# ETH3D/dataset-pipeline

Hardware: AMD Instinct MI355X
Metric: ICP correspondences/sec (higher is better)
Workload: dtype f32 (f64 accumulation); 1 GPU; ICPScanAligner 2 scans x 50000000 points, -d 0.01 (BASELINE.json configs[1] shape), one outer iteration per step; scans=2, parallelism=dp1

## Files before the change

### dataset-pipeline_amd/csrc/e3d_icp.hip

```cpp
#include <atomic>
#include <algorithm>
#include <cfloat>
#include <chrono>
#include <cmath>
#include <condition_variable>
#include <cstdio>
#include <functional>
#include <map>
#include <memory>
#include <mutex>
#include <thread>

#include "../../include/e3d_hip.h"
#include "e3d_comm.hpp"
#include "e3d_icp_kernels.hpp"
#include "e3d_math.hpp"

#pragma clang fp contract(off)

namespace e3d {

static thread_local std::string g_last_error;
void set_last_error(const std::string& msg) { g_last_error = msg; }
const char* last_error_cstr() { return g_last_error.c_str(); }
// ... 123 lines not shown
  bool stop_ = false;
};

}

using namespace e3d;

struct e3d_icp {
  int device = 0;
  hipStream_t stream = nullptr;
  std::vector<std::unique_ptr<Cloud>> clouds;
  std::unique_ptr<Cloud> fixed;
  int max_inner = 150;
  bool sequential_dsum = env_default_off("E3D_ICP_SEQUENTIAL_DISTANCE_SUM");
  DevBuf<float> d2_by_orig;
  std::vector<float> h_d2_by_orig;
  int nn_mode = 0;
  size_t dense_cell_budget = [] { const char* e = getenv("E3D_DENSE_CELLS"); return e ? (size_t)strtoull(e, nullptr, 10) : (size_t)1 << 33; }();
  int rank = 0, world = 1;
  e3d_allreduce_fn allreduce = nullptr;
  void* allreduce_user = nullptr;
  e3d_comm* comm = nullptr;
  DevBuf<double> d_red;

  DevBuf<float> bbox_partial, bbox_out;
  PinBuf<float> h_bbox;
  DevBuf<unsigned long long> keys_a, keys_b;
  DevBuf<unsigned> vals_a, vals_b, counter;
  DevBuf<char> sort_temp;
  DevBuf<int> match_pos;
  DevBuf<float> match_d2;
  DevBuf<unsigned> block_counts, block_offsets, block_groups, chunk_groups;
  DevBuf<unsigned char> block_done;
  DevBuf<double> block_d2, chunk_d2;
  DevBuf<unsigned long long> d_total, chunk_sum;
  DevBuf<double> d_total_d2;
  PinBuf<unsigned long long> h_total;
  PinBuf<double> h_total_d2;
  DevBuf<float4> cA, cB, cC;
  size_t corr_used = 0;
  bool resident_rows = env_default_on("E3D_ICP_RESIDENT");
  bool resident_now = false;
  int lm_prev_end_step = -1;
  std::unique_ptr<SolvePool> solve_pool;
  DevBuf<LmSet> d_sets;
  PinBuf<LmSet> h_sets;
  DevBuf<LmPose> d_poses;
  PinBuf<LmPose> h_poses;
  DevBuf<int> d_block_set;
  DevBuf<double> d_partial, d_setsum;
  PinBuf<double> h_setsum;
  std::unique_ptr<EventTimer> lm_timer, nn_timer, nn_timer_c;
  struct LazyTimer {
    std::vector<std::pair<hipEvent_t, hipEvent_t>> ev;
    size_t used = 0;
    double acc = 0.0;
    void start(hipStream_t s) {
      if (used == ev.size()) { hipEvent_t a, b; E3D_HIP(hipEventCreate(&a)); E3D_HIP(hipEventCreate(&b)); ev.emplace_back(a, b); }
      E3D_HIP(hipEventRecord(ev[used].first, s));
    }
    void stop(hipStream_t s) { E3D_HIP(hipEventRecord(ev[used].second, s)); ++used; }
    double take() {
      for (size_t i = 0; i < used; ++i) {
        float t = 0.f;
        if (hipEventSynchronize(ev[i].second) == hipSuccess && hipEventElapsedTime(&t, ev[i].first, ev[i].second) == hipSuccess) acc += (double)t;
      }
// ... 459 lines not shown
  if (kept == 0) return 0;
  if (k32) sort_pairs_u32_u32(reinterpret_cast<unsigned*>(h->keys_a.p), reinterpret_cast<unsigned*>(h->keys_b.p), h->vals_a.p, h->vals_b.p, kept, tgt.key_bits, h->sort_temp, s, n);
  else sort_pairs_u64_u32(h->keys_a.p, h->keys_b.p, h->vals_a.p, h->vals_b.p, kept, tgt.key_bits, h->sort_temp, s, n);
  return kept;
}

static double g_nn_prof[8];
static bool nn_profile() { static const bool on = env_default_off("E3D_NN_PROFILE"); return on; }
struct NnPhase {
  hipStream_t s; int slot; std::chrono::steady_clock::time_point t0;
  NnPhase(hipStream_t st, int sl) : s(st), slot(sl) { if (nn_profile()) { (void)hipStreamSynchronize(s); t0 = std::chrono::steady_clock::now(); } }
  ~NnPhase() { if (nn_profile()) { (void)hipStreamSynchronize(s); g_nn_prof[slot] += std::chrono::duration<double, std::milli>(std::chrono::steady_clock::now() - t0).count(); } }
};

static bool pair_is_dense(const e3d_icp* h, const Cloud& tgt) {
  return h->nn_mode >= 2 || (h->nn_mode == 0 && (double)tgt.n >= 4.0 * (double)std::max(tgt.n_cells, 1u));
}
static bool pair_uses_rows(const e3d_icp* h, const Cloud& tgt) {
  return pair_is_dense(h, tgt) && tgt.has_dense && (h->nn_mode == 0 || h->nn_mode == 3 || h->nn_mode == 5);
}
static bool far_list_is_short(size_t n_far, size_t n) {
  static const long long div = [] { const char* e = getenv("E3D_NN_FAR_DIV"); return e ? atoll(e) : 32ll; }();
  return n_far > 0 && (div <= 0 || n_far * (size_t)div < n);
}
static size_t resident_rows_cap(size_t n) { return div_up(n, 64) * 64; }
static size_t resident_bytes(size_t n) { return resident_rows_cap(n) * 48 + n * 4 + div_up(n, 64) * 4; }

struct BatchItem {
  PairJob* job; Cloud* src; Cloud* tgt; size_t j0, n; PairState* ps;
  InvMap im; CertParams cert; BoundParams bp; double cum_pair;
  MotionBound cum_up;
  float near2; bool none_near;
  bool certified = false, from_state = false; size_t n_near = 0, n_far = 0;
};

static void prepare_pair(BatchItem& it, float d) {
  const NnSwitches& sw = nn_switches();
  const Cloud& src = *it.src; const Cloud& tgt = *it.tgt;
  const PairState& ps = *it.ps;
  it.im = make_invmap(tgt);
  it.cum_pair = src.cum_motion + tgt.cum_motion;
  MotionBound m_lo;
  pair_motion_bounds(ps, src, tgt, m_lo, it.cum_up);
  it.cert = make_cert_params(tgt, m_lo);
  it.n_far = it.n; it.n_near = 0;
  it.certified = !ps.fresh && sw.use_cert && certify_now(ps, src, tgt);
  it.from_state = !ps.fresh && sw.use_cert && !it.certified;
  it.near2 = (float)((sw.near_frac * (double)d) * (sw.near_frac * (double)d));
  it.none_near = sw.np_frac > 0 && (src.last_motion + tgt.last_motion) < sw.np_gate * (double)d;
  double smin = cloud_smin(tgt);
  if (!(smin > 1e-12)) smin = 1e-12;
  double m_local = 0;
  for (int k = 0; k < 3; ++k) m_local = std::max(m_local, std::max(std::fabs((double)tgt.lmin[k]), std::fabs((double)tgt.lmax[k])));
  it.bp.margin = (float)(sw.margin_frac * (double)d);
  it.bp.rho_scale = round_up_f((1.0 + 1e-5) / smin);
  it.bp.rho_pad = round_up_f(2.0 * tgt.build_slack + 8.0 * FLT_EPSILON * m_local);
  it.bp.lo = it.cert.lo;
  it.bp.cell_scale = it.cert.cell_scale; it.bp.cell_sub = it.cert.cell_sub;
  it.bp.np_extra = it.none_near ? (float)(sw.np_frac * (double)d) : 0.f;
}

static void search_bounded_lists(e3d_icp* h, BatchItem& it, const unsigned* todo_near, const unsigned* todo_far, float* match_d2, float d, e3d_icp_iter_record& rec) {
  hipStream_t s = h->stream;
  const Cloud& tgt = *it.tgt;
  PairState& ps = *it.ps;
  const float4* srcG = it.src->G4.p + it.j0;
// ... 270 lines not shown
    launch_corr_totals(n, h->block_counts.p, h->block_d2.p, h->block_groups.p, h->chunk_sum.p, h->chunk_d2.p, h->chunk_groups.p,
                       h->d_totals_all.p + 3 * i, h->d_d2_all.p + i, ps.glist.p, s);
    h->tm_scan.stop(s);
    rec.nn_update_launches++; rec.nn_kernel_launches += 4;
  }
  read_back_batch(h, items, rec);
}

static bool find_pairs_multi(e3d_icp* h, std::vector<BatchItem>& items, float d, e3d_icp_iter_record& rec) {
  hipStream_t s = h->stream;
  const size_t B = items.size();
  for (const BatchItem& it : items) if (!it.tgt->has_half || h->nn_mode == 5) return false;
  const NnSwitches& sw = nn_switches();
  while (h->slots.size() < B) h->slots.emplace_back(new e3d_icp::PairSlot());
  h->h_todo_all.reserve(2 * kPairBatch); h->d_todo_all.reserve(2 * kPairBatch);
  h->d_totals_all.reserve(3 * kPairBatch); h->d_d2_all.reserve(kPairBatch); h->h_totals_all.reserve(3 * kPairBatch); h->h_d2_all.reserve(kPairBatch);
  h->h_batch.reserve(1); h->d_batch.reserve(1);
  NnBatchDev& T = h->h_batch.p[0];
  static_assert(kPairBatch <= (size_t)kNnBatchPairs, "pair table too small");
  T.n_pairs = (int)B; T.n_jobs = 0;
  unsigned cert_blocks = 0, upd_blocks = 0, chunks = 0;
  long long cert_queries = 0;
  E3D_HIP(hipMemsetAsync(h->d_todo_all.p, 0, 2 * sizeof(unsigned) * B, s));
  for (size_t i = 0; i < B; ++i) {
    BatchItem& it = items[i];
    e3d_icp::PairSlot& sl = *h->slots[i];
    Cloud& src = *it.src; Cloud& tgt = *it.tgt;
    PairState& ps = *it.ps;
    const size_t n = it.n;
    sl.match_d2.reserve(n); sl.todo_near.reserve(n); sl.todo_far.reserve(n);
    prepare_pair(it, d);
    const RowFrames rf = ensure_resident_rows(ps, src, tgt, n, s);
    const bool sg = rf.sg, tg = rf.tg;
    NnPairDev& P = T.pair[i];
    P.Gsrc = src.G4.p + it.j0; P.Gtgt = tgt.G4.p; P.S = tgt.dense_start.p; P.H8 = tgt.half_prefix.p;
    P.match = ps.match.p; P.match2 = ps.match2.p; P.lbe = ps.lbe.p; P.match_d2 = sl.match_d2.p;
    P.todo_near = sl.todo_near.p; P.todo_far = sl.todo_far.p; P.counts = h->d_todo_all.p + 2 * i;
    P.n = (unsigned)n; P.none_near = it.none_near ? 1 : 0;
    P.cum_up = it.cum_up;
    P.near2 = it.near2;
    P.g = tgt.grid; P.im = it.im; P.qr = tgt.qrange; P.bp = it.bp;
    P.Psrc = (sg ? src.G4.p : src.L4.p) + it.j0; P.LNsrc = src.LN.p + it.j0; P.Ptgt = tg ? tgt.G4.p : tgt.L4.p; P.LNtgt = tgt.LN.p;
    P.src_global = sg ? 1 : 0; P.tgt_global = tg ? 1 : 0; P.Tsrc = to_affine(src.T); P.Ttgt = to_affine(tgt.T);
    P.A = ps.pA.p; P.B = ps.pB.p; P.C = ps.pC.p; P.plane_match = ps.plane_match.p; P.glist = ps.glist.p;
    if (it.certified) { cert_blocks += (unsigned)div_up(n, (size_t)kNnCertBlockQueries); cert_queries += (long long)n; }
    T.cert_end[i] = cert_blocks;
    const unsigned nb = (unsigned)div_up(n, kBlock);
    upd_blocks += nb; T.upd_end[i] = upd_blocks;
    chunks += (unsigned)div_up((size_t)nb, (size_t)kNnScanChunk); T.chunk_end[i] = chunks;
  }
  h->block_counts.reserve(upd_blocks); h->block_d2.reserve(upd_blocks); h->block_groups.reserve(upd_blocks);
  h->chunk_sum.reserve(chunks + 1); h->chunk_d2.reserve(chunks + 1); h->chunk_groups.reserve(chunks + 1); h->chunk_rewritten.reserve(chunks + 1);
  {
    if (sw.fuse_update && cert_blocks) { h->block_done.reserve(upd_blocks); E3D_HIP(hipMemsetAsync(h->block_done.p, 0, upd_blocks, s)); }
    unsigned b0 = 0;
    for (size_t i = 0; i < B; ++i) {
      NnPairDev& P = T.pair[i];
      const bool on = sw.fuse_update && cert_blocks && items[i].certified && (1.0 - items[i].ps->settled_frac) < sw.fuse_gate;
      P.upd_counts = on ? h->block_counts.p + b0 : nullptr; P.upd_d2 = on ? h->block_d2.p + b0 : nullptr;
      P.upd_groups = on ? h->block_groups.p + b0 : nullptr; P.upd_done = on ? h->block_done.p + b0 : nullptr;
      b0 = T.upd_end[i];
    }
  }
  E3D_HIP(hipMemcpyAsync(h->d_batch.p, h->h_batch.p, sizeof(NnBatchDev), hipMemcpyHostToDevice, s));
  if (cert_blocks) {
    h->tm_certify.start(s);
    launch_nn_certify_multi(h->d_batch.p, cert_blocks, radius_sq(d), s);
    h->tm_certify.stop(s);
    rec.nn_certify_launches++; rec.nn_certify_queries += cert_queries; rec.nn_kernel_launches++;
    copy_out(h->h_todo_all.p, h->d_todo_all.p, 2 * sizeof(unsigned) * B, s);
  }
  sync(h);
  unsigned job_blocks = 0;
  long long job_queries = 0;
  for (size_t i = 0; i < B; ++i) {
    BatchItem& it = items[i];
    if (!it.certified) continue;
    e3d_icp::PairSlot& sl = *h->slots[i];
    it.n_near = h->h_todo_all.p[2 * i]; it.n_far = h->h_todo_all.p[2 * i + 1];
    certify_ran(*it.ps, *it.src, *it.tgt, it.n, it.n_near + it.n_far);
    auto add_job = [&](const unsigned* list, size_t n_list) {
      if (!n_list) return;
      const int jb = T.n_jobs++;
      T.job_pair[jb] = (int)i; T.job_list[jb] = list; T.job_n[jb] = (unsigned)n_list;
      job_blocks += (unsigned)div_up(n_list, kBlock); T.job_end[jb] = job_blocks;
      job_queries += (long long)n_list;
    };
    add_job(sl.todo_near.p, it.n_near);
    if (far_list_is_short(it.n_far, it.n)) {
      add_job(sl.todo_far.p, it.n_far);
      it.n_near += it.n_far; it.n_far = 0;
    }
  }
  auto launch_bounded_jobs = [&] {
    if (T.n_jobs <= 0) return;
    E3D_HIP(hipMemcpyAsync(h->d_batch.p, h->h_batch.p, sizeof(NnBatchDev), hipMemcpyHostToDevice, s));
    h->tm_bounded.start(s);
    launch_nn_bounded_half_multi(h->d_batch.p, job_blocks, radius_sq(d), s);
    h->tm_bounded.stop(s);
    rec.nn_bounded_launches++; rec.nn_bounded_queries += job_queries; rec.nn_kernel_launches++;
  };
  auto seeds_for = [&](const BatchItem& it) { return sw.seed_allowed && it.n_far > 0 && (it.ps->fresh ? sw.seed_fresh : it.ps->matched_frac >= sw.seed_frac); };
  size_t far_pairs = 0, far_total = 0;
  int kb_max = 1;
  for (size_t i = 0; i < B; ++i) if (items[i].n_far > 0) { ++far_pairs; far_total += items[i].n_far; kb_max = std::max(kb_max, items[i].tgt->key_bits); }
// ... 960 lines not shown
```

### dataset-pipeline_amd/csrc/e3d_icp_kernels.hip

```cpp
#include <cstdlib>

#include "e3d_icp_kernels.hpp"

#pragma clang fp contract(off)

namespace e3d {

__global__ __launch_bounds__(kBlock) void k_transform_aos(const float* __restrict__ xyz,
                                                          const float* __restrict__ nrm, size_t n, Affine T,
                                                          float* __restrict__ oxyz, float* __restrict__ onrm,
                                                          float* __restrict__ bbox_partial) {
  float mn[3] = {3.402823466e+38f, 3.402823466e+38f, 3.402823466e+38f};
  float mx[3] = {-3.402823466e+38f, -3.402823466e+38f, -3.402823466e+38f};
  for (size_t i = (size_t)blockIdx.x * blockDim.x + threadIdx.x; i < n; i += (size_t)gridDim.x * blockDim.x) {
    const float x = xyz[3 * i], y = xyz[3 * i + 1], z = xyz[3 * i + 2];
    const float3 p = pcl_se3(T, x, y, z);
    oxyz[3 * i] = p.x; oxyz[3 * i + 1] = p.y; oxyz[3 * i + 2] = p.z;
    if (nrm) {
      const float3 q = pcl_so3(T, nrm[3 * i], nrm[3 * i + 1], nrm[3 * i + 2]);
      onrm[3 * i] = q.x; onrm[3 * i + 1] = q.y; onrm[3 * i + 2] = q.z;
    }
    mn[0] = fminf(mn[0], p.x); mn[1] = fminf(mn[1], p.y); mn[2] = fminf(mn[2], p.z);
    mx[0] = fmaxf(mx[0], p.x); mx[1] = fmaxf(mx[1], p.y); mx[2] = fmaxf(mx[2], p.z);
  }
// ... 1074 lines not shown
        for (int r = 0; r < 9; ++r) {
          if (Q[G].bt - p < rl[r]) lb_pos = (int)(rs[r] + (Q[G].bt - p));
          p += rl[r];
        }
      }
      float lb_d2 = Q[G].bd; unsigned lb_oi = Q[G].boi;
      {
        const float od2 = __shfl_xor(lb_d2, 32, 64);
        const unsigned ooi = (unsigned)__shfl_xor((int)lb_oi, 32, 64);
        const int opos = __shfl_xor(lb_pos, 32, 64);
        if (od2 < lb_d2 || (od2 == lb_d2 && ooi < lb_oi)) { lb_d2 = od2; lb_oi = ooi; lb_pos = opos; }
      }
      const float sd2 = __shfl(lb_d2, slot_of_lane & 31, 64);
      const unsigned soi = (unsigned)__shfl((int)lb_oi, slot_of_lane & 31, 64);
      const int spos = __shfl(lb_pos, slot_of_lane & 31, 64);
      if ((slot_of_lane >> 5) == G) { rd2 = sd2; roi = soi; rpos = spos; }
    }
    if ((seg >> lane) & 1ull) {
      if (rd2 < best_d2 || (rd2 == best_d2 && roi < best_oi)) { best_d2 = rd2; best_oi = roi; best_pos = rpos; }
    }
    remaining &= ~seg;
  }
  if (valid) { match_pos[pos] = best_pos; match_d2[pos] = best_d2; }
}

constexpr int kCertPerWave = 512;
template <int kCertUnroll>
__device__ __forceinline__ void nn_certify_body(const unsigned bx, const float4* __restrict__ Gsrc, size_t n, const float4* __restrict__ Gtgt,
                                                const MotionBound cum_up, float r2, float near2, int none_near, int* __restrict__ match,
                                                int* __restrict__ match2, const float* __restrict__ lbe,
                                                float* __restrict__ match_d2, unsigned* __restrict__ todo_near,
                                                unsigned* __restrict__ todo_far, unsigned* __restrict__ counts,
                                                unsigned* __restrict__ upd_counts = nullptr, double* __restrict__ upd_d2 = nullptr,
                                                unsigned* __restrict__ upd_groups = nullptr, unsigned char* __restrict__ upd_done = nullptr) {
  __shared__ unsigned s_list[2][kBlock / kWave][kCertPerWave];
  __shared__ unsigned s_cnt[2][kBlock / kWave];
  __shared__ unsigned s_base[2];
  const int lane = threadIdx.x & 63, w = threadIdx.x >> 6;
  const size_t j0 = ((size_t)bx * (kBlock / kWave) + (size_t)w) * kCertPerWave;
  unsigned cn = 0, cf = 0;
  for (int step0 = 0; step0 < kCertPerWave / kWave; step0 += kCertUnroll) {
    size_t jj[kCertUnroll];
    bool vv[kCertUnroll];
    int mm[kCertUnroll], mm2[kCertUnroll];
    float ll[kCertUnroll];
    float4 qq[kCertUnroll], c1[kCertUnroll], c2v[kCertUnroll];
#pragma unroll
    for (int u = 0; u < kCertUnroll; ++u) {
      jj[u] = j0 + (size_t)(step0 + u) * kWave + (size_t)lane;
      vv[u] = jj[u] < n;
      const size_t js = vv[u] ? jj[u] : 0;
      mm[u] = ld_stream(match + js); mm2[u] = ld_stream(match2 + js); ll[u] = ld_stream(lbe + js); qq[u] = ld_stream(Gsrc + js);
    }
#pragma unroll
    for (int u = 0; u < kCertUnroll; ++u) {
      c1[u] = Gtgt[mm[u] >= 0 ? mm[u] : 0];
      c2v[u] = Gtgt[(mm[u] >= 0 && mm2[u] >= 0) ? mm2[u] : 0];
    }
    unsigned ub_c = 0, ub_g = 0, ub_gm = 0;
    double ub_t = 0.0;
    bool ub_bad = false;
    static_assert(kCertUnroll == 4, "four steps of 64 queries = one block of the row update");
#pragma unroll
    for (int u = 0; u < kCertUnroll; ++u) {
    const size_t j = jj[u];
    const bool valid = vv[u];
    bool ok = false, near = false;
    bool swapped = false;
    float v_ok = 0.f;
    if (valid) {
      const float thr = (ll[u] - motion_up(qq[u], cum_up)) * 0.999999f;
      const float lim = thr * thr * 0.999999f;
      const int m = mm[u];
      if (m >= 0) {
        const int m2 = mm2[u];
        const float4 q = qq[u];
        const float4 c = c1[u];
        float v = sqdist_l2(q.x, q.y, q.z, c.x, c.y, c.z);
        if (m2 >= 0) {
          const float4 c2 = c2v[u];
          const float v2 = sqdist_l2(q.x, q.y, q.z, c2.x, c2.y, c2.z);
          if (v2 < v || (v2 == v && __float_as_uint(c2.w) < __float_as_uint(c.w))) {
            v = v2;
            if (thr > 0.f && v < lim && v < r2) { match[j] = m2; match2[j] = m; swapped = true; }
          }
        }
        ok = (thr > 0.f) && (v < lim) && (v < r2);
        near = v < near2;
        if (ok) { st_stream(match_d2 + j, v); v_ok = v; }
      } else {
        ok = (thr > 0.f) && (lim >= r2);
        near = none_near != 0;
        st_stream(match_d2 + j, r2);
      }
    }
    const unsigned long long fn = __ballot(valid && !ok && near), ff = __ballot(valid && !ok && !near);
    const unsigned long long below = (1ull << lane) - 1ull;
    if (valid && !ok) {
      if (near) s_list[0][w][cn + (unsigned)__popcll(fn & below)] = (unsigned)j;
      else s_list[1][w][cf + (unsigned)__popcll(ff & below)] = (unsigned)j | (mm[u] < 0 ? kListNoPartner : 0u);
    }
    cn += (unsigned)__popcll(fn); cf += (unsigned)__popcll(ff);
    if (upd_done) {
      const bool f = valid && mm[u] >= 0;
      const unsigned gc = (unsigned)__popcll(__ballot(f));
      const double gd = wave_sum((f && ok) ? (double)v_ok : 0.0);
      ub_c += gc; ub_t += gd;
      if (gc) { ++ub_g; ub_gm |= 1u << u; }
      if (__ballot(valid && (!ok || swapped))) ub_bad = true;
    }
    }
    if (upd_done) {
      const size_t blk = j0 / kBlock + (size_t)(step0 / kCertUnroll);
      if (blk < (n + kBlock - 1) / kBlock && lane == 0) {
        if (!ub_bad) { upd_counts[blk] = ub_c; upd_d2[blk] = ub_t; upd_groups[blk] = ub_g | (ub_gm << 8); }
        upd_done[blk] = ub_bad ? 0 : 1;
      }
    }
  }
  if (lane == 0) { s_cnt[0][w] = cn; s_cnt[1][w] = cf; }
  __syncthreads();
  if (threadIdx.x < 2) {
    unsigned tot = 0;
    for (int k = 0; k < kBlock / kWave; ++k) tot += s_cnt[threadIdx.x][k];
    s_base[threadIdx.x] = tot ? atomicAdd(&counts[threadIdx.x], tot) : 0u;
  }
  __syncthreads();
  unsigned bn = s_base[0], bf = s_base[1];
  for (int k = 0; k < w; ++k) { bn += s_cnt[0][k]; bf += s_cnt[1][k]; }
  for (unsigned i = (unsigned)lane; i < cn; i += kWave) todo_near[bn + i] = s_list[0][w][i];
  for (unsigned i = (unsigned)lane; i < cf; i += kWave) todo_far[bf + i] = s_list[1][w][i];
}

template <int kCertUnroll>
__global__ __launch_bounds__(kBlock) void k_nn_certify(const float4* __restrict__ Gsrc, size_t n, const float4* __restrict__ Gtgt,
                                                       MotionBound cum_up, float r2, float near2, int none_near, int* __restrict__ match,
                                                       int* __restrict__ match2, const float* __restrict__ lbe,
                                                       float* __restrict__ match_d2, unsigned* __restrict__ todo_near,
                                                       unsigned* __restrict__ todo_far, unsigned* __restrict__ counts) {
  nn_certify_body<kCertUnroll>(blockIdx.x, Gsrc, n, Gtgt, cum_up, r2, near2, none_near, match, match2, lbe, match_d2, todo_near, todo_far, counts);
}

__device__ __forceinline__ int nn_find_range(const unsigned* __restrict__ ends, int n, unsigned b) {
  int lo = 0, hi = n - 1;
  while (lo < hi) {
    const int mid = (lo + hi) >> 1;
    if (b < ends[mid]) hi = mid; else lo = mid + 1;
  }
  return __builtin_amdgcn_readfirstlane(lo);
}

__global__ __launch_bounds__(kBlock) void k_nn_certify_multi(const NnBatchDev* __restrict__ B, float r2) {
  const int p = nn_find_range(B->cert_end, B->n_pairs, blockIdx.x);
  const unsigned bx = blockIdx.x - (p ? B->cert_end[p - 1] : 0u);
  const NnPairDev& P = B->pair[p];
  nn_certify_body<4>(bx, P.Gsrc, (size_t)P.n, P.Gtgt, P.cum_up, r2, P.near2, P.none_near, P.match, P.match2, P.lbe, P.match_d2,
                     P.todo_near, P.todo_far, P.counts, P.upd_counts, P.upd_d2, P.upd_groups, P.upd_done);
}

template <int LPQ>
__global__ __launch_bounds__(kBlock) void k_nn_bounded(const float4* __restrict__ Gsrc, const unsigned* __restrict__ list,
                                                       unsigned n_list, const float4* __restrict__ Gtgt, const unsigned* __restrict__ S,
                                                       GridDesc g, InvMap im, QueryRange qr, float r2, BoundParams bp,
                                                       int* __restrict__ match, int* __restrict__ match2,
                                                       float* __restrict__ match_d2, float* __restrict__ lbe) {
  const unsigned i = (blockIdx.x * blockDim.x + threadIdx.x) / LPQ;
  const int sub = threadIdx.x % LPQ;
  if (i >= n_list) return;
  const unsigned j = list[i] & kListIndexMask;
  const float4 q = Gsrc[j];
  const int m = match[j];
  float d1 = r2;
  if (m >= 0) {
    const float4 pc = Gtgt[m];
    d1 = sqdist_l2(q.x, q.y, q.z, pc.x, pc.y, pc.z);
    const int m2 = match2[j];
    if (m2 >= 0) { const float4 pc2 = Gtgt[m2]; d1 = fminf(d1, sqdist_l2(q.x, q.y, q.z, pc2.x, pc2.y, pc2.z)); }
  }
  const float dr = sqrtf(fminf(d1, r2)) + ((m < 0) ? bp.np_extra : bp.margin);
  const float cover2 = (d1 < r2) ? fminf(dr * dr * 1.000001f, r2) : ((m < 0) ? dr * dr * 1.000001f : r2);
  const float rho = sqrtf(cover2) * bp.rho_scale + bp.rho_pad;
  const float dx = q.x - im.t[0], dy = q.y - im.t[1], dz = q.z - im.t[2];
  const float lx = im.Linv[0] * dx + im.Linv[1] * dy + im.Linv[2] * dz;
  const float ly = im.Linv[3] * dx + im.Linv[4] * dy + im.Linv[5] * dz;
  const float lz = im.Linv[6] * dx + im.Linv[7] * dy + im.Linv[8] * dz;
  const int x0 = max(cell_coord(lx - rho, g.origin[0], g.inv_cell) - qr.lo[0], 0), x1 = min(cell_coord(lx + rho, g.origin[0], g.inv_cell) - qr.lo[0], (int)qr.D[0] - 1);
  const int y0 = max(cell_coord(ly - rho, g.origin[1], g.inv_cell) - qr.lo[1], 0), y1 = min(cell_coord(ly + rho, g.origin[1], g.inv_cell) - qr.lo[1], (int)qr.D[1] - 1);
  const int z0 = max(cell_coord(lz - rho, g.origin[2], g.inv_cell) - qr.lo[2], 0), z1 = min(cell_coord(lz + rho, g.origin[2], g.inv_cell) - qr.lo[2], (int)qr.D[2] - 1);
  const float kInf = __uint_as_float(0x7f800000u);
  float cover_box2 = 0.f;
// ... 620 lines not shown
                                                         float4* __restrict__ C, size_t out_base) {
  const size_t j = (size_t)blockIdx.x * blockDim.x + threadIdx.x;
  const int m = (j < n) ? ld_stream(match_pos + j) : -1;
  const bool f = m >= 0;
  const unsigned long long b = __ballot(f);
  __shared__ unsigned wbase[kBlock / kWave];
  const int lane = threadIdx.x & 63, w = threadIdx.x >> 6;
  if (lane == 0) wbase[w] = (unsigned)__popcll(b);
  __syncthreads();
  unsigned base = block_offsets[blockIdx.x];
  for (int k = 0; k < w; ++k) base += wbase[k];
  if (!f) return;
  const unsigned rank = (unsigned)__popcll(b & ((1ull << lane) - 1ull));
  const size_t o = out_base + base + rank;
  const size_t js = order ? (size_t)ld_stream(order + j) : j;
  const float4 sp = order ? Gsrc[js] : ld_stream(Gsrc + js);
  const float4 ln = order ? LNsrc[js] : ld_stream(LNsrc + js);
  const float3 sn = pcl_so3(Tsrc, ln.x, ln.y, ln.z);
  const float4 tp = Gtgt[m];
  const float4 tl = LNtgt[m];
  const float3 tn = pcl_so3(Ttgt, tl.x, tl.y, tl.z);
  st_stream(A + o, make_float4(sp.x, sp.y, sp.z, sn.x));
  st_stream(B + o, make_float4(sn.y, sn.z, tp.x, tp.y));
  st_stream(C + o, make_float4(tp.z, tn.x, tn.y, tn.z));
}

__device__ __forceinline__ void corr_update_body(const unsigned bx, const int* __restrict__ match, int* __restrict__ plane_match,
                                                 const float* __restrict__ match_d2, size_t n,
                                                 const float4* __restrict__ Psrc, const float4* __restrict__ LNsrc,
                                                 const int src_global, const Affine& Tsrc, const float4* __restrict__ Ptgt,
                                                 const float4* __restrict__ LNtgt, const int tgt_global, const Affine& Ttgt,
                                                 float4* __restrict__ A, float4* __restrict__ B, float4* __restrict__ C,
                                                 unsigned* __restrict__ block_counts, double* __restrict__ block_d2,
                                                 unsigned* __restrict__ block_groups, const unsigned char* __restrict__ done = nullptr) {
  if (done && done[bx]) return;
  const size_t j = (size_t)bx * blockDim.x + threadIdx.x;
  const bool in = j < n;
  const int m = in ? ld_stream(match + j) : -1;
  const int pm = in ? ld_stream(plane_match + j) : -1;
  const bool f = m >= 0;
  const unsigned long long chg = __ballot(in && m != pm);
  const bool wr = in && (((chg >> (threadIdx.x & 56)) & 0xFFull) != 0ull);
  const unsigned long long wrb = __ballot(wr);
  if (wr) {
    float4 ra = make_float4(0.f, 0.f, 0.f, 0.f), rb = ra, rc = ra;
    if (f) {
      const float4 sp = Psrc[j];
      const float4 ln = LNsrc[j];
      float3 sn = make_float3(ln.x, ln.y, ln.z);
      if (src_global) sn = pcl_so3(Tsrc, ln.x, ln.y, ln.z);
      const float4 tp = Ptgt[m];
      const float4 tl = LNtgt[m];
      float3 tn = make_float3(tl.x, tl.y, tl.z);
      if (tgt_global) tn = pcl_so3(Ttgt, tl.x, tl.y, tl.z);
      ra = make_float4(sp.x, sp.y, sp.z, sn.x);
      rb = make_float4(sn.y, sn.z, tp.x, tp.y);
      rc = make_float4(tp.z, tn.x, tn.y, tn.z);
    }
    st_stream(A + j, ra); st_stream(B + j, rb); st_stream(C + j, rc);
    if (m != pm) plane_match[j] = m;
  }
  const unsigned long long b = __ballot(f);
  double d = f ? (double)ld_stream(match_d2 + j) : 0.0;
  d = wave_sum(d);
  __shared__ unsigned sc[kBlock / kWave], sw[kBlock / kWave];
  __shared__ double sd[kBlock / kWave];
  if ((threadIdx.x & 63) == 0) { sc[threadIdx.x >> 6] = (unsigned)__popcll(b); sw[threadIdx.x >> 6] = (unsigned)__popcll(wrb); sd[threadIdx.x >> 6] = d; }
  __syncthreads();
  if (threadIdx.x == 0) {
    unsigned c = 0, g = 0, gm = 0, rw = 0; double t = 0;
    for (int k = 0; k < kBlock / kWave; ++k) { c += sc[k]; t += sd[k]; rw += sw[k]; if (sc[k]) { ++g; gm |= 1u << k; } }
    block_counts[bx] = c; block_d2[bx] = t; block_groups[bx] = g | (gm << 8) | (rw << 16);
  }
}

__global__ __launch_bounds__(kBlock) void k_corr_update(const int* __restrict__ match, int* __restrict__ plane_match,
                                                        const float* __restrict__ match_d2, size_t n,
                                                        const float4* __restrict__ Psrc, const float4* __restrict__ LNsrc,
                                                        const int src_global, Affine Tsrc, const float4* __restrict__ Ptgt,
                                                        const float4* __restrict__ LNtgt, const int tgt_global, Affine Ttgt,
                                                        float4* __restrict__ A, float4* __restrict__ B, float4* __restrict__ C,
                                                        unsigned* __restrict__ block_counts, double* __restrict__ block_d2,
                                                        unsigned* __restrict__ block_groups) {
  corr_update_body(blockIdx.x, match, plane_match, match_d2, n, Psrc, LNsrc, src_global, Tsrc, Ptgt, LNtgt, tgt_global, Ttgt, A, B, C,
                   block_counts, block_d2, block_groups);
}

__global__ __launch_bounds__(kBlock) void k_corr_update_multi(const NnBatchDev* __restrict__ Bt, unsigned* __restrict__ block_counts,
                                                              double* __restrict__ block_d2, unsigned* __restrict__ block_groups) {
  const int p = nn_find_range(Bt->upd_end, Bt->n_pairs, blockIdx.x);
  const unsigned b0 = p ? Bt->upd_end[p - 1] : 0u;
  const NnPairDev& P = Bt->pair[p];
  const Affine Ts = P.Tsrc, Tt = P.Ttgt;
  corr_update_body(blockIdx.x - b0, P.match, P.plane_match, P.match_d2, (size_t)P.n, P.Psrc, P.LNsrc, P.src_global, Ts, P.Ptgt, P.LNtgt,
                   P.tgt_global, Tt, P.A, P.B, P.C, block_counts + b0, block_d2 + b0, block_groups + b0, P.upd_done);
}

__device__ __forceinline__ void group_list_body(const unsigned bx, const unsigned* __restrict__ block_groups, int nblocks,
                                                const unsigned* __restrict__ chunk_gbase, unsigned* __restrict__ glist) {
  const int b = (int)bx * kScanChunk + threadIdx.x;
  const unsigned w = (b < nblocks) ? block_groups[b] : 0u;
  const unsigned c = w & 0xFFu;
  const int lane = threadIdx.x & 63, wv = threadIdx.x >> 6;
  unsigned inc = c;
#pragma unroll
  for (int o = 1; o < 64; o <<= 1) {
    const unsigned t = __shfl_up(inc, o, 64);
    if (lane >= o) inc += t;
  }
  __shared__ unsigned ws[kScanChunk / kWave];
  if (lane == 63) ws[wv] = inc;
  __syncthreads();
  unsigned base = chunk_gbase[bx] + (inc - c);
  for (int k = 0; k < wv; ++k) base += ws[k];
  const unsigned mask = w >> 8;
#pragma unroll
  for (int k = 0; k < kBlock / kWave; ++k)
    if (mask & (1u << k)) glist[base++] = (unsigned)b * (kBlock / kWave) + (unsigned)k;
}

__global__ __launch_bounds__(kScanChunk) void k_group_list(const unsigned* __restrict__ block_groups, int nblocks,
                                                           const unsigned* __restrict__ chunk_gbase,
                                                           unsigned* __restrict__ glist) {
  group_list_body(blockIdx.x, block_groups, nblocks, chunk_gbase, glist);
}

__global__ __launch_bounds__(kScanChunk) void k_scan_chunk_sums_multi(const NnBatchDev* __restrict__ Bt, const unsigned* __restrict__ block_counts,
                                                                      const double* __restrict__ block_d2, const unsigned* __restrict__ block_groups,
// ... 874 lines not shown
```

### dataset-pipeline_amd/csrc/e3d_icp_kernels.hpp

```cpp
#pragma once

#include <functional>

#include "e3d_common.hpp"
#include "e3d_kernels.hpp"

namespace e3d {

enum { kModeCost = 0,
       kModeOne = 1,
       kModeTwo = 2,
       kModeTwoCross = 3
};
constexpr int kLmMaxPoses = 10;
constexpr int kLmSlot = 91;
constexpr int kMaxBboxBlocks = 2048;
constexpr int kRowCap = 128;
constexpr unsigned kListNoPartner = 0x80000000u, kListIndexMask = 0x7FFFFFFFu;
constexpr int kRowSpan = 4;
constexpr int kNNCap = 256;

struct QueryRange { int lo[3]; unsigned D[3]; };

struct LmSet {
// ... 61 lines not shown
  float rho_scale;
  float rho_pad;
  MotionBound lo;
  float cell_scale, cell_sub;
  float np_extra;
};
void launch_nn_bounded(const float4* Gsrc, const unsigned* list, size_t n_list, const float4* Gtgt, const unsigned* dense_start,
                       const unsigned long long* half_prefix, bool half_always, const GridDesc& g, const InvMap& im, const QueryRange& qr, float r2,
                       const BoundParams& bp, int* match, int* match2, float* match_d2, float* lbe, hipStream_t s);
constexpr int kNnBatchPairs = 32;
constexpr int kNnBatchJobs = 2 * kNnBatchPairs;
struct NnPairDev {
  const float4* Gsrc;
  const float4* Gtgt;
  const unsigned* S;
  const unsigned long long* H8;
  int *match, *match2;
  float* lbe;
  float* match_d2;
  unsigned *todo_near, *todo_far;
  unsigned* counts;
  unsigned n;
  int none_near;
  MotionBound cum_up;
  float near2;
  GridDesc g; InvMap im; QueryRange qr; BoundParams bp;
  const float4 *Psrc, *LNsrc, *Ptgt, *LNtgt;
  int src_global, tgt_global;
  Affine Tsrc, Ttgt;
  float4 *A, *B, *C;
  int* plane_match;
  unsigned* glist;
  unsigned* upd_counts; double* upd_d2; unsigned* upd_groups; unsigned char* upd_done;
  const unsigned* far_list;
  const unsigned* occ;
  unsigned far_n, occ_stride;
  int far_flags;
  unsigned rows_off, rows_n;
  unsigned* seed_list;
  float seed2;
};
constexpr unsigned kQueryKeysBlock = 2048;
constexpr unsigned kQuerySeedBlock = 1024;
struct NnBatchDev {
  int n_pairs, n_jobs;
  int key_shift;
  unsigned far_end[kNnBatchPairs];
  unsigned rows_end[kNnBatchPairs];
  unsigned cert_end[kNnBatchPairs];
  unsigned upd_end[kNnBatchPairs];
  unsigned chunk_end[kNnBatchPairs];
  unsigned job_end[kNnBatchJobs];
  int job_pair[kNnBatchJobs];
  unsigned job_n[kNnBatchJobs];
  const unsigned* job_list[kNnBatchJobs];
  NnPairDev pair[kNnBatchPairs];
};
void launch_nn_certify_multi(const NnBatchDev* batch, unsigned n_blocks, float r2, hipStream_t s);
void launch_nn_bounded_half_multi(const NnBatchDev* batch, unsigned n_blocks, float r2, hipStream_t s);
void launch_query_keys_multi(bool keys32, const NnBatchDev* batch, unsigned n_blocks, float r2, void* keys, unsigned* vals, unsigned* counts, hipStream_t s);
void launch_query_seed_multi(bool keys32, const NnBatchDev* batch, unsigned n_blocks, float r2, void* keys, unsigned* vals, unsigned* counts, hipStream_t s);
void launch_nn_rows_multi(const NnBatchDev* batch, unsigned n_blocks, const unsigned* order, float r2, hipStream_t s);
void launch_corr_update_multi(const NnBatchDev* batch, unsigned n_blocks, unsigned* block_counts, double* block_d2, unsigned* block_groups, hipStream_t s);
void launch_corr_totals_multi(const NnBatchDev* batch, int n_pairs, unsigned n_chunks, const unsigned* block_counts, const double* block_d2,
                              const unsigned* block_groups, unsigned long long* chunk_sum, double* chunk_d2, unsigned* chunk_groups,
                              unsigned* chunk_rewritten, unsigned long long* totals, double* total_d2, hipStream_t s);
// ... 43 lines not shown
```

Measured before the change: 6.719 billion correspondences/s.

## Settle fused row-update work per wave instead of per block

The certify kernel now records which of the four 64-query waves in a row-update block are settled, storing per-wave counts and d2 sums for partially settled blocks instead of marking the whole block unsettled. The row-update kernel skips loads and stores for settled waves and reads their precomputed stats, so mixed blocks do less work. It also disables fusion for pairs whose resident rows were just reset, and adds an optional stats dump of how many blocks are settled whole or mixed. This costs extra scratch buffers and per-wave branching inside the update kernel.

```diff
diff --git a/dataset-pipeline_amd/csrc/e3d_icp.hip b/dataset-pipeline_amd/csrc/e3d_icp.hip
--- a/dataset-pipeline_amd/csrc/e3d_icp.hip
+++ b/dataset-pipeline_amd/csrc/e3d_icp.hip
@@ -179,6 +179,8 @@
   DevBuf<float> match_d2;
   DevBuf<unsigned> block_counts, block_offsets, block_groups, chunk_groups;
   DevBuf<unsigned char> block_done;
+  DevBuf<unsigned> block_gcnt;
+  DevBuf<double> block_gd2;
   DevBuf<double> block_d2, chunk_d2;
   DevBuf<unsigned long long> d_total, chunk_sum;
   DevBuf<double> d_total_d2;
@@ -704,6 +706,7 @@
   MotionBound cum_up;
   float near2; bool none_near;
   bool certified = false, from_state = false; size_t n_near = 0, n_far = 0;
+  bool rows_reset = false;
 };
 
 static void prepare_pair(BatchItem& it, float d) {
@@ -1040,6 +1043,7 @@
     prepare_pair(it, d);
     const RowFrames rf = ensure_resident_rows(ps, src, tgt, n, s);
     const bool sg = rf.sg, tg = rf.tg;
+    it.rows_reset = rf.reset;
     NnPairDev& P = T.pair[i];
     P.Gsrc = src.G4.p + it.j0; P.Gtgt = tgt.G4.p; P.S = tgt.dense_start.p; P.H8 = tgt.half_prefix.p;
     P.match = ps.match.p; P.match2 = ps.match2.p; P.lbe = ps.lbe.p; P.match_d2 = sl.match_d2.p;
@@ -1060,13 +1064,17 @@
   h->block_counts.reserve(upd_blocks); h->block_d2.reserve(upd_blocks); h->block_groups.reserve(upd_blocks);
   h->chunk_sum.reserve(chunks + 1); h->chunk_d2.reserve(chunks + 1); h->chunk_groups.reserve(chunks + 1); h->chunk_rewritten.reserve(chunks + 1);
   {
-    if (sw.fuse_update && cert_blocks) { h->block_done.reserve(upd_blocks); E3D_HIP(hipMemsetAsync(h->block_done.p, 0, upd_blocks, s)); }
+    if (sw.fuse_update && cert_blocks) {
+      h->block_done.reserve(upd_blocks); h->block_gcnt.reserve(upd_blocks); h->block_gd2.reserve(4 * (size_t)upd_blocks);
+      E3D_HIP(hipMemsetAsync(h->block_done.p, 0, upd_blocks, s));
+    }
     unsigned b0 = 0;
     for (size_t i = 0; i < B; ++i) {
       NnPairDev& P = T.pair[i];
-      const bool on = sw.fuse_update && cert_blocks && items[i].certified && (1.0 - items[i].ps->settled_frac) < sw.fuse_gate;
+      const bool on = sw.fuse_update && cert_blocks && items[i].certified && !items[i].rows_reset && (1.0 - items[i].ps->settled_frac) < sw.fuse_gate;
       P.upd_counts = on ? h->block_counts.p + b0 : nullptr; P.upd_d2 = on ? h->block_d2.p + b0 : nullptr;
       P.upd_groups = on ? h->block_groups.p + b0 : nullptr; P.upd_done = on ? h->block_done.p + b0 : nullptr;
+      P.upd_gcnt = on ? h->block_gcnt.p + b0 : nullptr; P.upd_gd2 = on ? h->block_gd2.p + 4 * (size_t)b0 : nullptr;
       b0 = T.upd_end[i];
     }
   }
@@ -1079,6 +1087,23 @@
     copy_out(h->h_todo_all.p, h->d_todo_all.p, 2 * sizeof(unsigned) * B, s);
   }
   sync(h);
+  if (sw.want_stats && sw.fuse_update && cert_blocks) {
+    std::vector<unsigned char> masks(upd_blocks);
+    E3D_HIP(hipMemcpyAsync(masks.data(), h->block_done.p, upd_blocks, hipMemcpyDeviceToHost, s));
+    sync(h);
+    unsigned b0 = 0;
+    for (size_t i = 0; i < B; ++i) {
+      unsigned whole = 0, mixed = 0, groups = 0;
+      for (unsigned b = b0; b < T.upd_end[i]; ++b) {
+        const unsigned m = masks[b];
+        if (m == 0xFu) ++whole; else if (m) ++mixed;
+        groups += (unsigned)__builtin_popcount(m);
+      }
+      if (T.pair[i].upd_done)
+        fprintf(stderr, "[fuse %d->%d] blocks %u settled whole %u mixed %u settled groups %u\n", items[i].job->src, items[i].job->tgt, T.upd_end[i] - b0, whole, mixed, groups);
+      b0 = T.upd_end[i];
+    }
+  }
   unsigned job_blocks = 0;
   long long job_queries = 0;
   for (size_t i = 0; i < B; ++i) {
diff --git a/dataset-pipeline_amd/csrc/e3d_icp_kernels.hip b/dataset-pipeline_amd/csrc/e3d_icp_kernels.hip
--- a/dataset-pipeline_amd/csrc/e3d_icp_kernels.hip
+++ b/dataset-pipeline_amd/csrc/e3d_icp_kernels.hip
@@ -1130,7 +1130,8 @@
                                                 float* __restrict__ match_d2, unsigned* __restrict__ todo_near,
                                                 unsigned* __restrict__ todo_far, unsigned* __restrict__ counts,
                                                 unsigned* __restrict__ upd_counts = nullptr, double* __restrict__ upd_d2 = nullptr,
-                                                unsigned* __restrict__ upd_groups = nullptr, unsigned char* __restrict__ upd_done = nullptr) {
+                                                unsigned* __restrict__ upd_groups = nullptr, unsigned char* __restrict__ upd_done = nullptr,
+                                                unsigned* __restrict__ upd_gcnt = nullptr, double* __restrict__ upd_gd2 = nullptr) {
   __shared__ unsigned s_list[2][kBlock / kWave][kCertPerWave];
   __shared__ unsigned s_cnt[2][kBlock / kWave];
   __shared__ unsigned s_base[2];
@@ -1155,9 +1156,8 @@
       c1[u] = Gtgt[mm[u] >= 0 ? mm[u] : 0];
       c2v[u] = Gtgt[(mm[u] >= 0 && mm2[u] >= 0) ? mm2[u] : 0];
     }
-    unsigned ub_c = 0, ub_g = 0, ub_gm = 0;
-    double ub_t = 0.0;
-    bool ub_bad = false;
+    unsigned ub_m = 0, ub_pc = 0;
+    double ub_d[kCertUnroll];
     static_assert(kCertUnroll == 4, "four steps of 64 queries = one block of the row update");
 #pragma unroll
     for (int u = 0; u < kCertUnroll; ++u) {
@@ -1199,20 +1199,33 @@
       else s_list[1][w][cf + (unsigned)__popcll(ff & below)] = (unsigned)j | (mm[u] < 0 ? kListNoPartner : 0u);
     }
     cn += (unsigned)__popcll(fn); cf += (unsigned)__popcll(ff);
-    if (upd_done) {
+    ub_d[u] = 0.0;
+    if (upd_done && !__ballot(valid && (!ok || swapped))) {
       const bool f = valid && mm[u] >= 0;
-      const unsigned gc = (unsigned)__popcll(__ballot(f));
-      const double gd = wave_sum((f && ok) ? (double)v_ok : 0.0);
-      ub_c += gc; ub_t += gd;
-      if (gc) { ++ub_g; ub_gm |= 1u << u; }
-      if (__ballot(valid && (!ok || swapped))) ub_bad = true;
+      ub_pc |= (unsigned)__popcll(__ballot(f)) << (8 * u);
+      ub_d[u] = wave_sum(f ? (double)v_ok : 0.0);
+      ub_m |= 1u << u;
     }
     }
     if (upd_done) {
       const size_t blk = j0 / kBlock + (size_t)(step0 / kCertUnroll);
       if (blk < (n + kBlock - 1) / kBlock && lane == 0) {
-        if (!ub_bad) { upd_counts[blk] = ub_c; upd_d2[blk] = ub_t; upd_groups[blk] = ub_g | (ub_gm << 8); }
-        upd_done[blk] = ub_bad ? 0 : 1;
+        if (ub_m == 0xFu) {
+          unsigned c = 0, g = 0, gm = 0; double t = 0;
+#pragma unroll
+          for (int u = 0; u < kCertUnroll; ++u) {
+            const unsigned gc = (ub_pc >> (8 * u)) & 0xFFu;
+            c += gc; t += ub_d[u];
+            if (gc) { ++g; gm |= 1u << u; }
+          }
+          upd_counts[blk] = c; upd_d2[blk] = t; upd_groups[blk] = g | (gm << 8);
+        } else if (ub_m) {
+          upd_gcnt[blk] = ub_pc;
+#pragma unroll
+          for (int u = 0; u < kCertUnroll; ++u)
+            if (ub_m & (1u << u)) upd_gd2[4 * blk + (size_t)u] = ub_d[u];
+        }
+        upd_done[blk] = (unsigned char)ub_m;
       }
     }
   }
@@ -1253,7 +1266,7 @@
   const unsigned bx = blockIdx.x - (p ? B->cert_end[p - 1] : 0u);
   const NnPairDev& P = B->pair[p];
   nn_certify_body<4>(bx, P.Gsrc, (size_t)P.n, P.Gtgt, P.cum_up, r2, P.near2, P.none_near, P.match, P.match2, P.lbe, P.match_d2,
-                     P.todo_near, P.todo_far, P.counts, P.upd_counts, P.upd_d2, P.upd_groups, P.upd_done);
+                     P.todo_near, P.todo_far, P.counts, P.upd_counts, P.upd_d2, P.upd_groups, P.upd_done, P.upd_gcnt, P.upd_gd2);
 }
 
 template <int LPQ>
@@ -1940,40 +1953,47 @@
                                                  const float4* __restrict__ LNtgt, const int tgt_global, const Affine& Ttgt,
                                                  float4* __restrict__ A, float4* __restrict__ B, float4* __restrict__ C,
                                                  unsigned* __restrict__ block_counts, double* __restrict__ block_d2,
-                                                 unsigned* __restrict__ block_groups, const unsigned char* __restrict__ done = nullptr) {
-  if (done && done[bx]) return;
-  const size_t j = (size_t)bx * blockDim.x + threadIdx.x;
-  const bool in = j < n;
-  const int m = in ? ld_stream(match + j) : -1;
-  const int pm = in ? ld_stream(plane_match + j) : -1;
-  const bool f = m >= 0;
-  const unsigned long long chg = __ballot(in && m != pm);
-  const bool wr = in && (((chg >> (threadIdx.x & 56)) & 0xFFull) != 0ull);
-  const unsigned long long wrb = __ballot(wr);
-  if (wr) {
-    float4 ra = make_float4(0.f, 0.f, 0.f, 0.f), rb = ra, rc = ra;
-    if (f) {
-      const float4 sp = Psrc[j];
-      const float4 ln = LNsrc[j];
-      float3 sn = make_float3(ln.x, ln.y, ln.z);
-      if (src_global) sn = pcl_so3(Tsrc, ln.x, ln.y, ln.z);
-      const float4 tp = Ptgt[m];
-      const float4 tl = LNtgt[m];
-      float3 tn = make_float3(tl.x, tl.y, tl.z);
-      if (tgt_global) tn = pcl_so3(Ttgt, tl.x, tl.y, tl.z);
-      ra = make_float4(sp.x, sp.y, sp.z, sn.x);
-      rb = make_float4(sn.y, sn.z, tp.x, tp.y);
-      rc = make_float4(tp.z, tn.x, tn.y, tn.z);
-    }
-    st_stream(A + j, ra); st_stream(B + j, rb); st_stream(C + j, rc);
-    if (m != pm) plane_match[j] = m;
-  }
-  const unsigned long long b = __ballot(f);
-  double d = f ? (double)ld_stream(match_d2 + j) : 0.0;
-  d = wave_sum(d);
+                                                 unsigned* __restrict__ block_groups, const unsigned char* __restrict__ done = nullptr,
+                                                 const unsigned* __restrict__ gcnt = nullptr, const double* __restrict__ gd2 = nullptr) {
+  const unsigned settled = done ? (unsigned)done[bx] : 0u;
+  if (settled == 0xFu) return;
   __shared__ unsigned sc[kBlock / kWave], sw[kBlock / kWave];
   __shared__ double sd[kBlock / kWave];
-  if ((threadIdx.x & 63) == 0) { sc[threadIdx.x >> 6] = (unsigned)__popcll(b); sw[threadIdx.x >> 6] = (unsigned)__popcll(wrb); sd[threadIdx.x >> 6] = d; }
+  const int wv = __builtin_amdgcn_readfirstlane((int)(threadIdx.x >> 6));
+  if ((settled >> wv) & 1u) {
+    if ((threadIdx.x & 63) == 0) { sc[wv] = (gcnt[bx] >> (8 * wv)) & 0xFFu; sw[wv] = 0u; sd[wv] = gd2[4 * (size_t)bx + (size_t)wv]; }
+  } else {
+    const size_t j = (size_t)bx * blockDim.x + threadIdx.x;
+    const bool in = j < n;
+    const int m = in ? ld_stream(match + j) : -1;
+    const int pm = in ? ld_stream(plane_match + j) : -1;
+    const bool f = m >= 0;
+    const unsigned long long chg = __ballot(in && m != pm);
+    const bool wr = in && (((chg >> (threadIdx.x & 56)) & 0xFFull) != 0ull);
+    const unsigned long long wrb = __ballot(wr);
+    if (wr) {
+      float4 ra = make_float4(0.f, 0.f, 0.f, 0.f), rb = ra, rc = ra;
+      if (f) {
+        const float4 sp = Psrc[j];
+        const float4 ln = LNsrc[j];
+        float3 sn = make_float3(ln.x, ln.y, ln.z);
+        if (src_global) sn = pcl_so3(Tsrc, ln.x, ln.y, ln.z);
+        const float4 tp = Ptgt[m];
+        const float4 tl = LNtgt[m];
+        float3 tn = make_float3(tl.x, tl.y, tl.z);
+        if (tgt_global) tn = pcl_so3(Ttgt, tl.x, tl.y, tl.z);
+        ra = make_float4(sp.x, sp.y, sp.z, sn.x);
+        rb = make_float4(sn.y, sn.z, tp.x, tp.y);
+        rc = make_float4(tp.z, tn.x, tn.y, tn.z);
+      }
+      st_stream(A + j, ra); st_stream(B + j, rb); st_stream(C + j, rc);
+      if (m != pm) plane_match[j] = m;
+    }
+    const unsigned long long b = __ballot(f);
+    double d = f ? (double)ld_stream(match_d2 + j) : 0.0;
+    d = wave_sum(d);
+    if ((threadIdx.x & 63) == 0) { sc[wv] = (unsigned)__popcll(b); sw[wv] = (unsigned)__popcll(wrb); sd[wv] = d; }
+  }
   __syncthreads();
   if (threadIdx.x == 0) {
     unsigned c = 0, g = 0, gm = 0, rw = 0; double t = 0;
@@ -2001,7 +2021,7 @@
   const NnPairDev& P = Bt->pair[p];
   const Affine Ts = P.Tsrc, Tt = P.Ttgt;
   corr_update_body(blockIdx.x - b0, P.match, P.plane_match, P.match_d2, (size_t)P.n, P.Psrc, P.LNsrc, P.src_global, Ts, P.Ptgt, P.LNtgt,
-                   P.tgt_global, Tt, P.A, P.B, P.C, block_counts + b0, block_d2 + b0, block_groups + b0, P.upd_done);
+                   P.tgt_global, Tt, P.A, P.B, P.C, block_counts + b0, block_d2 + b0, block_groups + b0, P.upd_done, P.upd_gcnt, P.upd_gd2);
 }
 
 __device__ __forceinline__ void group_list_body(const unsigned bx, const unsigned* __restrict__ block_groups, int nblocks,
diff --git a/dataset-pipeline_amd/csrc/e3d_icp_kernels.hpp b/dataset-pipeline_amd/csrc/e3d_icp_kernels.hpp
--- a/dataset-pipeline_amd/csrc/e3d_icp_kernels.hpp
+++ b/dataset-pipeline_amd/csrc/e3d_icp_kernels.hpp
@@ -117,6 +117,7 @@
   int* plane_match;
   unsigned* glist;
   unsigned* upd_counts; double* upd_d2; unsigned* upd_groups; unsigned char* upd_done;
+  unsigned* upd_gcnt; double* upd_gd2;
   const unsigned* far_list;
   const unsigned* occ;
   unsigned far_n, occ_stride;
```

Measured after the change: 6.700 billion correspondences/s. Within noise of the previous version (-0.3%).
